# leggedrobotics/traversability_estimation

Measured on NVIDIA H100. Metric: Mcells/s full filter chain, synthetic elevation, higher is better.
Workload: dtype f32 (f64 certified slow path)

## Files before the change

### traversability_estimation_b200/csrc/te_capi.cu

```cuda
#include <cuda.h>
#include <cuda_runtime.h>

#include <cmath>
#include <cstdarg>
#include <cstdio>
#include <cstring>
#include <functional>
#include <map>
#include <mutex>
#include <string>
#include <vector>

#include "../../include/te_b200.h"
#include "te_kernels.h"
#include "te_fused.h"
#include "te_footprint.h"

namespace {

thread_local std::string g_last_error;

int fail(int code, const char* fmt, ...) {
  char buf[512];
  va_list ap;
// ... 207 lines not shown
  return TE_OK;
}

template <class F>
cudaError_t for_wrapped_pieces(int rows, int cols, int sr, int sc, int c0, int n, F&& copy) {
  for (int done = 0; done < n;) {
    const int c = c0 + done, js = (c + sc) % cols;
    const int m = std::min(n - done, cols - js);
    const size_t d = (size_t)c * rows, h = (size_t)js * rows;
    cudaError_t e = copy(d, h + sr, rows - sr, m);
    if (e == cudaSuccess && sr > 0) e = copy(d + (rows - sr), h, sr, m);
    if (e != cudaSuccess) return e;
    done += m;
  }
  return cudaSuccess;
}

cudaError_t upload_cols(float* dev, const float* host, int rows, int cols, int sr, int sc, int c0, int n, cudaStream_t s) {
  const size_t pitch = sizeof(float) * (size_t)rows;
  if (sr == 0 && sc == 0) return cudaMemcpyAsync(dev + (size_t)c0 * rows, host + (size_t)c0 * rows, pitch * n, cudaMemcpyHostToDevice, s);
  return for_wrapped_pieces(rows, cols, sr, sc, c0, n, [&](size_t d, size_t h, int r, int m) {
    return cudaMemcpy2DAsync(dev + d, pitch, host + h, pitch, sizeof(float) * r, m, cudaMemcpyHostToDevice, s);
  });
}

cudaError_t download_cols(float* host, const float* dev, int rows, int cols, int sr, int sc, int c0, int n, cudaStream_t s) {
  const size_t pitch = sizeof(float) * (size_t)rows;
  if (sr == 0 && sc == 0) return cudaMemcpyAsync(host + (size_t)c0 * rows, dev + (size_t)c0 * rows, pitch * n, cudaMemcpyDeviceToHost, s);
  return for_wrapped_pieces(rows, cols, sr, sc, c0, n, [&](size_t d, size_t h, int r, int m) {
    return cudaMemcpy2DAsync(host + h, pitch, dev + d, pitch, sizeof(float) * r, m, cudaMemcpyDeviceToHost, s);
  });
}

struct Staging {
  te_ctx* c;
  bool host;
  int rows, cols, sr, sc;
  int rc = TE_OK;
  int used = 0;
  struct Out { void* host; const void* dev; size_t bytes; int ncols; };
  Out outs[sizeof(te_ctx::stage) / sizeof(DevBuf)];
  int nout = 0;

  Staging(te_ctx* ctx, bool host_memory, const te_geometry* g)
      : c(ctx), host(host_memory), rows(g->rows), cols(g->cols), sr(g->start_row), sc(g->start_col) {}

  void check(cudaError_t e, const char* what) {
    if (rc == TE_OK && e != cudaSuccess) rc = fail(TE_ERR_CUDA, "%s failed: %s", what, cudaGetErrorString(e));
  }
  void* slot(size_t bytes) {
    if (rc != TE_OK) return nullptr;
    if (used == (int)(sizeof(outs) / sizeof(outs[0]))) {
      rc = fail(TE_ERR_CUDA, "out of staging buffers");
      return nullptr;
    }
    DevBuf& b = c->stage[used++];
    check(b.reserve(std::max<size_t>(bytes, 1)), "staging allocation");
    return rc == TE_OK ? b.p : nullptr;
  }
  size_t layer_bytes(int ncols) const { return sizeof(float) * (size_t)rows * ncols; }
  const float* in_layer(const float* h, int ncols) {
    if (!host || !h) return h;
    float* d = (float*)slot(layer_bytes(ncols));
    if (d) check(upload_cols(d, h, rows, cols, sr, sc, 0, ncols, c->stream), "layer upload");
    return d;
  }
  template <class T>
  const T* in(const T* h, size_t n) {
    if (!host || !h) return h;
    T* d = (T*)slot(sizeof(T) * n);
    if (d && n) check(cudaMemcpyAsync(d, h, sizeof(T) * n, cudaMemcpyHostToDevice, c->stream), "upload");
    return d;
  }
  float* out_layer(float* h, int ncols) { return (float*)record(h, layer_bytes(ncols), ncols); }
  template <class T>
  T* out(T* h, size_t n) { return (T*)record(h, sizeof(T) * n, 0); }
  void* record(void* h, size_t bytes, int ncols) {
    if (!host || !h) return h;
    void* d = slot(bytes);
    if (d) outs[nout++] = Out{h, d, bytes, ncols};
    return d;
  }
  int finish() {
    if (!host || rc != TE_OK) return rc;
    for (int k = 0; k < nout; ++k) {
      const Out& o = outs[k];
      check(o.ncols ? download_cols((float*)o.host, (const float*)o.dev, rows, cols, sr, sc, 0, o.ncols, c->stream)
                    : cudaMemcpyAsync(o.host, o.dev, o.bytes, cudaMemcpyDeviceToHost, c->stream),
            "download");
    }
    check(cudaStreamSynchronize(c->stream), "cudaStreamSynchronize");
    return rc;
  }
};

int next_timing_slot(te_ctx* c, te_ctx::Ev3** out) {
  if (c->events_used == c->events.size()) {
    te_ctx::Ev3 ev{};
    TE_CUDA(cudaEventCreate(&ev.a)); TE_CUDA(cudaEventCreate(&ev.b)); TE_CUDA(cudaEventCreate(&ev.c));
    c->events.push_back(ev);
  }
  *out = &c->events[c->events_used];
  return TE_OK;
}

int run_chain_device(te_ctx* c, const te_geometry* g, const te::SlabView& v, const te_chain_params* p, const float* elev,
                     const te::ChainOut& o, int nmaps) {
  const te::ChainDev d = make_chain_dev(g, p);
  bool use_fused = false;
  if (c->kernel_choice != TE_KERNEL_GENERIC) {
    use_fused = te::fused_eligible(c->fused, c->hX, c->hY, g, p, c->stream);
    if (!use_fused && c->kernel_choice == TE_KERNEL_FUSED)
      return fail(TE_ERR_UNSUPPORTED, "fused stencil has no instantiation for these window shapes: %s", c->fused.why.c_str());
    if (use_fused) {
      if (const char* why = te::fused_launch_obstacle(v, nmaps, elev, o)) {
        if (c->kernel_choice == TE_KERNEL_FUSED) return fail(TE_ERR_UNSUPPORTED, "fused stencil cannot run this launch: %s", why);
        use_fused = false;
      }
    }
  }
  const size_t in_stride = (size_t)g->rows * v.in_ncols, out_stride = (size_t)g->rows * v.out_ncols;
  if (use_fused) {
    const size_t cells = out_stride * (size_t)nmaps;
    const size_t cap = te::fused_list_capacity(cells, c->sms);
    if (cap >= ((size_t)1 << 32)) return fail(TE_ERR_UNSUPPORTED, "launch of %zu cells exceeds the work-list index range", cells);
    TE_CUDA(c->worklist.reserve(sizeof(unsigned) * cap));
    TE_CUDA(c->worklist3.reserve(sizeof(unsigned) * cells));
    {
      const void* before = c->counter.p;
      TE_CUDA(c->counter.reserve(sizeof(unsigned) * 256));
      if (c->counter.p != before) c->counter_clean = -1;
    }
    {
      const te::ChainOut& om = o;
      const int phase = c->counter_phase ^ 1;
      unsigned* const cnt = (unsigned*)c->counter.p + 128 * phase;
      unsigned* const cnt_next = (unsigned*)c->counter.p + 128 * (phase ^ 1);
      if (c->counter_stream != c->stream) c->counter_clean = -1;
      c->counter_stream = c->stream;
      if (c->counter_clean != phase) TE_CUDA(cudaMemsetAsync(cnt, 0, sizeof(unsigned) * 128, c->stream));
      c->counter_clean = -1;
      c->counter_phase = phase;
      te_ctx::Ev3* ev = nullptr;
      if (c->timing) {
        if (int rc = next_timing_slot(c, &ev)) return rc;
        TE_CUDA(cudaEventRecord(ev->a, c->stream));
      }
      int rc = te::launch_chain_fused(c->fused, v, d, nmaps, elev, om, (unsigned*)c->worklist.p, cnt, (unsigned)cap, c->sms, c->stream);
      if (rc != 0) return fail(TE_ERR_CUDA, "fused chain launch failed: %s", c->fused.why.c_str());
      if (int r2 = launch_check(c, "k_chain_fused")) return r2;
      if (c->timing) TE_CUDA(cudaEventRecord(ev->b, c->stream));
      te::FixupArgs fa;
      te::make_fixup_args(c->fused, v, d, &fa);
      te::launch_fixup_t2(fa, elev, om, (const unsigned*)c->worklist.p, cnt, (unsigned)cap, (unsigned*)c->worklist3.p, cnt + 4,
                          (unsigned)cells, c->sms, c->stream, !c->timing);
      if (int r2 = launch_check(c, "k_fixup_t2")) return r2;
      te::launch_fixup(v, d, elev, om, (const unsigned*)c->worklist3.p, cnt + 4, (unsigned)cells, cnt_next, c->sms, c->stream, true);
      if (int r2 = launch_check(c, "k_fixup_cells")) return r2;
      c->counter_clean = phase ^ 1;
      if (c->timing) {
        TE_CUDA(cudaEventRecord(ev->c, c->stream));
        ++c->events_used;
      }
    }
  } else {
    for (int m = 0; m < nmaps; ++m) {
      te::ChainOut om = o;
      om.slope += m * out_stride; om.step += m * out_stride; om.rough += m * out_stride; om.trav += m * out_stride;
      if (om.nx) om.nx += m * out_stride;
      if (om.ny) om.ny += m * out_stride;
      if (om.nz) om.nz += m * out_stride;
      te_ctx::Ev3* ev = nullptr;
      if (c->timing) {
        if (int rc = next_timing_slot(c, &ev)) return rc;
        TE_CUDA(cudaEventRecord(ev->a, c->stream));
      }
      te::launch_chain_generic(v, d, elev + m * in_stride, om, c->sms, c->stream);
      if (int r2 = launch_check(c, "k_chain_generic")) return r2;
      if (c->timing) {
        TE_CUDA(cudaEventRecord(ev->b, c->stream));
        TE_CUDA(cudaEventRecord(ev->c, c->stream));
        ++c->events_used;
      }
    }
  }
  return TE_OK;
}

}

extern "C" {

int te_abi_version(void) { return TE_B200_ABI_VERSION; }

const char* te_last_error(void) { return g_last_error.c_str(); }

int te_create(te_ctx** out, int device) {
  if (!out) return fail(TE_ERR_BAD_ARG, "out pointer is null");
  *out = nullptr;
  int n = 0;
  cudaError_t e = cudaGetDeviceCount(&n);
  if (e != cudaSuccess || n <= 0)
    return fail(TE_ERR_CUDA, "no CUDA device available (%s); libte_b200 has no CPU fallback", e == cudaSuccess ? "device count 0" : cudaGetErrorString(e));
  if (device < 0 || device >= n) return fail(TE_ERR_BAD_ARG, "device %d out of range [0,%d)", device, n);
  int prev = 0;
  cudaGetDevice(&prev);
  TE_CUDA(cudaSetDevice(device));
  te_ctx* c = new te_ctx();
  c->device = device;
  cudaDeviceProp prop;
  if (cudaGetDeviceProperties(&prop, device) == cudaSuccess) c->sms = prop.multiProcessorCount;
  e = cudaStreamCreateWithFlags(&c->own_stream, cudaStreamNonBlocking);
  if (e != cudaSuccess) {
    delete c;
    cudaSetDevice(prev);
    return fail(TE_ERR_CUDA, "cudaStreamCreate failed: %s", cudaGetErrorString(e));
  }
  c->stream = c->own_stream;
  cudaSetDevice(prev);
  *out = c;
  return TE_OK;
}

int te_destroy(te_ctx* c) {
  if (!c) return TE_OK;
  {
    Guard g(c);
    if (g.ok) {
      cudaStreamSynchronize(c->stream);
      c->dX.release();
      c->dY.release();
      for (auto& b : c->stage) b.release();
      c->worklist.release();
      c->worklist3.release();
      c->counter.release();
      c->fused.release();
      c->fp.release();
      for (auto& e : c->events) { cudaEventDestroy(e.a); cudaEventDestroy(e.b); cudaEventDestroy(e.c); }
      if (c->s_h2d) cudaStreamDestroy(c->s_h2d);
      if (c->s_d2h) cudaStreamDestroy(c->s_d2h);
      if (c->own_stream) cudaStreamDestroy(c->own_stream);
    }
  }
  delete c;
  return TE_OK;
}

int te_host_alloc(void** out, size_t bytes) {
  if (!out) return fail(TE_ERR_BAD_ARG, "out pointer is null");
  *out = nullptr;
  TE_CUDA(cudaHostAlloc(out, bytes ? bytes : 1, cudaHostAllocDefault));
  return TE_OK;
}

int te_host_free(void* p) {
  if (!p) return TE_OK;
  TE_CUDA(cudaFreeHost(p));
  return TE_OK;
}

int te_set_stream(te_ctx* c, void* s) {
  TE_ENTER(c);
  c->stream = s ? (cudaStream_t)s : c->own_stream;
  return TE_OK;
}

int te_synchronize(te_ctx* c) {
  TE_ENTER(c);
  TE_CUDA(cudaStreamSynchronize(c->stream));
  return TE_OK;
}

int te_set_kernel(te_ctx* c, int choice) {
  TE_ENTER(c);
  if (choice < TE_KERNEL_AUTO || choice > TE_KERNEL_FUSED) return fail(TE_ERR_BAD_ARG, "unknown kernel choice %d", choice);
  c->kernel_choice = choice;
  return TE_OK;
}

int te_get_stats(te_ctx* c, int64_t* launches, int64_t* slow) {
  TE_ENTER(c);
  if (launches) *launches = c->launches;
  if (slow) {
    unsigned last[4] = {0, 0, 0, 0};
    if (c->counter.p) {
      TE_CUDA(cudaStreamSynchronize(c->stream));
      TE_CUDA(cudaMemcpy(last, (unsigned*)c->counter.p + 128 * c->counter_phase, sizeof(last), cudaMemcpyDeviceToHost));
    }
    *slow = (int64_t)last[1];
  }
  return TE_OK;
}

int te_enable_timing(te_ctx* c, int on) {
  TE_ENTER(c);
  c->timing = on != 0;
  return TE_OK;
}

int te_get_timing(te_ctx* c, double* main_ms, double* fixup_ms, int64_t* samples) {
  TE_ENTER(c);
  TE_CUDA(cudaStreamSynchronize(c->stream));
  double m = 0.0, f = 0.0;
  for (size_t k = 0; k < c->events_used; ++k) {
    const auto& e = c->events[k];
    float t1 = 0.f, t2 = 0.f;
    TE_CUDA(cudaEventElapsedTime(&t1, e.a, e.b));
    TE_CUDA(cudaEventElapsedTime(&t2, e.b, e.c));
// ... 1054 lines not shown
```

### traversability_estimation_b200/csrc/te_fixup.cu

```cuda
#include <algorithm>

#include "te_fused.h"

namespace te {
namespace {

struct Elev {
  const float* __restrict__ e;
  int rows, col0, ncols, cols_total;
  __device__ __forceinline__ float operator()(int a, int b) const {
    if (a < 0 || a >= rows || b < 0 || b >= cols_total) return nanf_();
    const int lb = b - col0;
    if (lb < 0 || lb >= ncols) return nanf_();
    const float v = __ldg(e + (size_t)lb * rows + a);
    return finitef(v) ? v : nanf_();
  }
};

__device__ float step_height_t2(const FixupArgs& A, const Elev& E, int a, int b) {
  const float zc = E(a, b);
  if (!finitef(zc)) return nanf_();
  const unsigned rm = A.rowmask ? A.rowmask[a] : 0u, cm = A.colmask ? A.colmask[b] : 0u;
  float mn = zc, mx = zc;
#pragma unroll
  for (int l = -2; l <= 2; ++l) {
    const int w = A.w1[l < 0 ? -l : l];
    for (int k = -w; k <= w; ++k) {
      const float z = E(a + k, b + l);
      if (finitef(z)) { mn = fminf(mn, z); mx = fmaxf(mx, z); }
    }
  }
  if (A.tip1) {
    const float t0 = (rm & 1u) ? E(a - 2, b) : nanf_(), t1 = (rm & 2u) ? E(a + 2, b) : nanf_();
    const float t2 = (cm & 1u) ? E(a, b - 2) : nanf_(), t3 = (cm & 2u) ? E(a, b + 2) : nanf_();
    mn = fminf(fminf(mn, t0), fminf(t1, fminf(t2, t3)));
    mx = fmaxf(fmaxf(mx, t0), fmaxf(t1, fmaxf(t2, t3)));
  }
  return (float)((double)mx - (double)mn);
}

__device__ __noinline__ float step_t2(const FixupArgs A, const Elev E, int i, int j) {
  const unsigned rm = A.rowmask ? A.rowmask[i] : 0u, cm = A.colmask ? A.colmask[j] : 0u;
  double stepMax = 0.0;
  int n = 0;
  bool any = false;
  auto visit = [&](int a, int b) {
    const float sh = step_height_t2(A, E, a, b);
    if (!finitef(sh)) return;
    any = true;
    if ((double)sh > stepMax) stepMax = (double)sh;
    if ((double)sh > A.step_crit) ++n;
  };
  for (int l = -2; l <= 2; ++l) {
    const int w = A.w2[l < 0 ? -l : l];
    for (int k = -w; k <= w; ++k) visit(i + k, j + l);
  }
  if (A.tip2) {
    if (rm & 4u) visit(i - 2, j);
    if (rm & 8u) visit(i + 2, j);
    if (cm & 4u) visit(i, j - 2);
    if (cm & 8u) visit(i, j + 2);
  }
  if (!any) return nanf_();
  const double step = fmin(stepMax, (double)n / (double)A.ncrit * stepMax);
  return (float)(step < A.step_crit ? 1.0 - step / A.step_crit : 0.0);
}

__constant__ double c_rcp[26] = {0.0,      1.0 / 1,  1.0 / 2,  1.0 / 3,  1.0 / 4,  1.0 / 5,  1.0 / 6,  1.0 / 7,  1.0 / 8,
                                 1.0 / 9,  1.0 / 10, 1.0 / 11, 1.0 / 12, 1.0 / 13, 1.0 / 14, 1.0 / 15, 1.0 / 16, 1.0 / 17,
                                 1.0 / 18, 1.0 / 19, 1.0 / 20, 1.0 / 21, 1.0 / 22, 1.0 / 23, 1.0 / 24, 1.0 / 25};

__device__ __forceinline__ float acos_t2(float x) {
  const float u = 1.0f - x;
  float p = fmaf(x, -0.0011488182935863733f, 0.006254698149859905f);
  p = fmaf(p, x, -0.016484638676047325f);
  p = fmaf(p, x, 0.03044925443828106f);
  p = fmaf(p, x, -0.05000271648168564f);
  p = fmaf(p, x, 0.08894557505846024f);
  p = fmaf(p, x, -0.21459604799747467f);
  p = fmaf(p, x, 1.570796251296997f);
  return sqrtf(u) * p;
}

constexpr unsigned shape_mask(int w0, int w1, int w2) {
  auto col = [](int w) { return w >= 2 ? 0x1fu : w == 1 ? 0x0eu : w == 0 ? 0x04u : 0u; };
  return (col(w2)) | (col(w1) << 5) | (col(w0) << 10) | (col(w1) << 15) | (col(w2) << 20);
}
constexpr unsigned SHAPE_A = shape_mask(2, 2, 1), SHAPE_B = shape_mask(1, 1, -1);

template <unsigned SHAPE>
__device__ bool normals_t2(const FixupArgs& A, const Elev& E, int i, int j, float& fnx, float& fny, float& fnz, float& slope,
                           float& rough, unsigned& why) {
  const float zc = E(i, j);
  if (!finitef(zc)) {
    fnx = fny = fnz = slope = rough = nanf_();
    return true;
  }
  unsigned mask = 0;
  double sw = 0, suw = 0, svw = 0, sww = 0;
  {
    const int lb0 = j - A.in_col0;
    const double dzc = (double)zc;
    unsigned shape = SHAPE;
    if (SHAPE == 0u) {
#pragma unroll
      for (int l = -2; l <= 2; ++l) {
        const int w = A.wn[l < 0 ? -l : l];
        shape |= (w >= 2 ? 0x1fu : w == 1 ? 0x0eu : w == 0 ? 0x04u : 0u) << ((l + 2) * 5);
      }
    }
    float v[5][5];
    if (i >= 2 && i + 2 < A.rows && j >= 2 && j + 2 < A.cols_total && lb0 >= 2 && lb0 + 2 < A.in_ncols) {
      const float* base = E.e + (size_t)lb0 * A.rows + i;
#pragma unroll
      for (int l = -2; l <= 2; ++l)
#pragma unroll
        for (int k = -2; k <= 2; ++k)
          v[l + 2][k + 2] = (SHAPE == 0u || ((SHAPE >> ((l + 2) * 5 + (k + 2))) & 1u)) ? __ldg(base + (ptrdiff_t)l * A.rows + k) : 0.0f;
    } else {
#pragma unroll
      for (int l = -2; l <= 2; ++l) {
        const int b = j + l, lb = lb0 + l;
        const bool col_ok = b >= 0 && b < A.cols_total && lb >= 0 && lb < A.in_ncols;
        const float* col = E.e + (size_t)min(max(lb, 0), A.in_ncols - 1) * A.rows;
#pragma unroll
        for (int k = -2; k <= 2; ++k) {
          const int a = i + k;
          if (SHAPE != 0u && !((SHAPE >> ((l + 2) * 5 + (k + 2))) & 1u)) { v[l + 2][k + 2] = 0.0f; continue; }
          const float x = __ldg(col + min(max(a, 0), A.rows - 1));
          v[l + 2][k + 2] = (col_ok && a >= 0 && a < A.rows) ? x : nanf_();
        }
      }
    }
#pragma unroll
    for (int l = -2; l <= 2; ++l) {
      double cs = 0.0, ck = 0.0;
#pragma unroll
      for (int k = -2; k <= 2; ++k) {
        const unsigned bitm = 1u << ((l + 2) * 5 + (k + 2));
        if (SHAPE != 0u && !(SHAPE & bitm)) continue;
        const bool ok = finitef(v[l + 2][k + 2]) && (shape & bitm) != 0u;
        mask |= ok ? bitm : 0u;
        const double d = (double)(ok ? v[l + 2][k + 2] : zc) - dzc;
        cs += d;
        if (k != 0) ck = fma((double)k, d, ck);
        sww = fma(d, d, sww);
      }
      sw += cs;
      suw += ck;
      if (l != 0) svw = fma((double)l, cs, svw);
    }
    suw *= -A.res;
    svw *= -A.res;
  }
  constexpr unsigned KM = 0x108421u, LM = 0x1fu;
  const int k_m2 = __popc(mask & KM), k_m1 = __popc(mask & (KM << 1)), k_p1 = __popc(mask & (KM << 3)), k_p2 = __popc(mask & (KM << 4));
  const int l_m2 = __popc(mask & LM), l_m1 = __popc(mask & (LM << 5)), l_p1 = __popc(mask & (LM << 15)), l_p2 = __popc(mask & (LM << 20));
  auto bit = [](int k, int l) { return 1u << ((l + 2) * 5 + (k + 2)); };
  const unsigned kl_p1 = bit(1, 1) | bit(-1, -1), kl_m1 = bit(1, -1) | bit(-1, 1);
  const unsigned kl_p2 = bit(2, 1) | bit(1, 2) | bit(-2, -1) | bit(-1, -2), kl_m2 = bit(2, -1) | bit(-1, 2) | bit(-2, 1) | bit(1, -2);
  const unsigned kl_p4 = bit(2, 2) | bit(-2, -2), kl_m4 = bit(2, -2) | bit(-2, 2);
  const int ik = 2 * (k_p2 - k_m2) + (k_p1 - k_m1), il = 2 * (l_p2 - l_m2) + (l_p1 - l_m1);
  const int ikk = 4 * (k_p2 + k_m2) + (k_p1 + k_m1), ill = 4 * (l_p2 + l_m2) + (l_p1 + l_m1);
  const int ikl = (__popc(mask & kl_p1) - __popc(mask & kl_m1)) + 2 * (__popc(mask & kl_p2) - __popc(mask & kl_m2)) +
                  4 * (__popc(mask & kl_p4) - __popc(mask & kl_m4));
  const double res2 = A.res * A.res;
  const int cnt = __popc(mask);
  const double su = -A.res * (double)ik, sv = -A.res * (double)il;
  const double suu = res2 * (double)ikk, svv = res2 * (double)ill, suv = res2 * (double)ikl;
  double nx = 0.0, ny = 0.0, nz = 1.0;
  const double rn = c_rcp[cnt];
  const double mu = su * rn, mv = sv * rn, mw = sw * rn;
  const double xx = fma(-su, mu, suu), xy = fma(-su, mv, suv), xz = fma(-su, mw, suw);
  const double yy = fma(-sv, mv, svv), yz = fma(-sv, mw, svw), zz = fma(-sw, mw, sww);
  if (cnt >= 3 && zz > 0.0) {
    double bx, by, bz;
    if (cnt == A.n_full_i) {
      const double a = 0.5 * (xx + yy), g2 = fma(xz, xz, yz * yz);
      const double h = 0.5 * (a - zz), hh = fma(h, h, g2);
      const double D = sqrt(hh);
      const double dph = D + fabs(h);
      why = 1u | ((unsigned)cnt << 8);
      if (!(dph > 0.0)) return false;
      const double qq = g2 / dph;
      const double m = h >= 0.0 ? dph : qq;
      const double lam = (h >= 0.0 ? zz : a) - qq;
      const double big = fmax(a, zz);
      why = 2u | ((unsigned)cnt << 8);
      if (!(lam > 1e-9 * big)) return false;
      why = 3u | ((unsigned)cnt << 8);
      if (!(fmin(2.0 * D, m) > 1e-7 * big)) return false;
      bx = -xz; by = -yz; bz = m;
    } else {
      const double c2 = xx + yy + zz;
      const double c1 = xx * yy + xx * zz + yy * zz - xy * xy - xz * xz - yz * yz;
      const double c0 = xx * (yy * zz - yz * yz) - xy * (xy * zz - yz * xz) + xz * (xy * yz - yy * xz);
      double lam = 0.0, dp = -c1;
      bool conv = false;
#pragma unroll 1
      for (int it = 0; it < 40; ++it) {
        const double pv = fma(fma(c2 - lam, lam, -c1), lam, c0);
        dp = fma(fma(-3.0, lam, 2.0 * c2), lam, -c1);
        const double hpp = fma(-3.0, lam, c2);
        const double den = fma(dp, dp, -pv * hpp);
        if (!(den > 0.0)) break;
        const double step = pv * dp / den;
        lam -= step;
        if (fabs(step) <= 1e-15 * c2) { conv = true; break; }
      }
      dp = fma(fma(-3.0, lam, 2.0 * c2), lam, -c1);
      why = (!conv ? 4u : !(lam > 1e-9 * c2) ? 5u : 6u) | ((unsigned)cnt << 8);
      if (!conv || !(lam > 1e-9 * c2) || !(fabs(dp) > 1e-4 * c2 * c2)) return false;
      const double ax = xx - lam, ay = yy - lam, az = zz - lam;
      const double v0x = xy * yz - xz * ay, v0y = xz * xy - ax * yz, v0z = ax * ay - xy * xy;
      const double v1x = xy * az - xz * yz, v1y = xz * xz - ax * az, v1z = ax * yz - xy * xz;
      const double v2x = ay * az - yz * yz, v2y = yz * xz - xy * az, v2z = xy * yz - ay * xz;
      const double q0 = v0x * v0x + v0y * v0y + v0z * v0z, q1 = v1x * v1x + v1y * v1y + v1z * v1z, q2 = v2x * v2x + v2y * v2y + v2z * v2z;
      bx = v0x; by = v0y; bz = v0z;
      double bq = q0;
      if (q1 > bq) { bx = v1x; by = v1y; bz = v1z; bq = q1; }
      if (q2 > bq) { bx = v2x; by = v2y; bz = v2z; bq = q2; }
    }
    const double bq = fma(bx, bx, fma(by, by, bz * bz));
    why = 7u | ((unsigned)cnt << 8);
    if (!(bq > 0.0)) return false;
    const double inv = rsqrt(bq);
    nx = bx * inv; ny = by * inv; nz = bz * inv;
    if (nz < 0.0) { nx = -nx; ny = -ny; nz = -nz; }
    why = 8u | ((unsigned)cnt << 8);
    if (nz == 0.0) return false;
    if (nz > 0.9998) {
      const float f = (float)nz;
      const float up = __uint_as_float(__float_as_uint(f) + 1u), dn = __uint_as_float(__float_as_uint(f) - 1u);
      const double bu = 0.5 * ((double)f + (double)up), bd = 0.5 * ((double)f + (double)dn);
      const double guard = A.nz_guard * (bu - bd);
      why = 9u | ((unsigned)cnt << 8);
      if (fabs(nz - bu) < guard || fabs(nz - bd) < guard) return false;
    }
  }
  fnx = (float)nx; fny = (float)ny; fnz = (float)nz;
  const double th = (double)acos_t2(fminf(fnz, 1.0f));
  slope = (float)(th < A.slope_crit ? fma(-th, A.inv_slope_crit, 1.0) : 0.0);
  const double NX = fnx, NY = fny, NZ = fnz;
  const double sum = fmax(NX * (NX * xx + 2.0 * (NY * xy + NZ * xz)) + NY * (NY * yy + 2.0 * NZ * yz) + NZ * NZ * zz, 0.0);
  if (cnt >= 2) {
    const double r = sqrt(sum * c_rcp[cnt - 1]);
    rough = (float)(r < A.rough_crit ? fma(-r, A.inv_rough_crit, 1.0) : 0.0);
  } else {
    rough = 0.0f;
  }
  return true;
}

template <unsigned SHAPE>
__global__ void __launch_bounds__(128, 8) k_fixup_t2(FixupArgs A, const float* __restrict__ elev, ChainOut o,
                                                  const unsigned* __restrict__ list, const unsigned* __restrict__ count,
                                                  unsigned cap, unsigned* list3, unsigned* count3, unsigned cap3) {
  asm volatile("griddepcontrol.launch_dependents;");
  asm volatile("griddepcontrol.wait;" ::: "memory");
  unsigned n = *count;
  if (n > cap) n = cap;
  for (unsigned k = blockIdx.x * blockDim.x + threadIdx.x; k < n; k += gridDim.x * blockDim.x) {
    const unsigned w = list[k];
    if (w == LIST_INVALID) continue;
    const unsigned c = w & 0x3fffffffu;
    const unsigned mapi = c / A.map_cells, cl = c - mapi * A.map_cells;
    const int i = (int)(cl % (unsigned)A.rows);
    const int j = A.out_col0 + (int)(cl / (unsigned)A.rows);
    const Elev E{elev + (size_t)mapi * A.in_map_stride, A.rows, A.in_col0, A.in_ncols, A.cols_total};
    const bool do_n = (w >> 30) & 1u, do_s = (w >> 31) & 1u;
    float s, r, t;
    bool escalate = false;
    unsigned why = 0;
    if (do_n) {
      float fx, fy, fz;
      if (normals_t2<SHAPE>(A, E, i, j, fx, fy, fz, s, r, why)) {
        o.slope[c] = s;
        o.rough[c] = r;
        if (o.nx) { o.nx[c] = fx; o.ny[c] = fy; o.nz[c] = fz; }
      } else {
        escalate = true;
      }
    } else {
      s = o.slope[c];
      r = o.rough[c];
    }
    if (do_s) {
      t = step_t2(A, E, i, j);
      o.step[c] = t;
    } else {
      t = o.step[c];
    }
    if (escalate) {
      const unsigned idx = atomicAdd(count3, 1u);
      if (idx < cap3) list3[idx] = c | (1u << 30);
      else atomicExch(count3 + 1, 1u);
      atomicAdd(count3 + 4 + (why & 15u), 1u);
      atomicAdd(count3 + 20 + min((why >> 8) & 31u, 25u), 1u);
    } else {
      o.trav[c] = __fmul_rn(A.fuse_w, __fadd_rn(__fadd_rn(s, t), r));
    }
  }
}

}

void launch_fixup_t2(const FixupArgs& a, const float* elev, const ChainOut& o, const unsigned* list, const unsigned* count,
                     unsigned cap, unsigned* list3, unsigned* count3, unsigned cap3, int sms, cudaStream_t s, bool pdl) {
  cudaLaunchConfig_t cfg{};
  const unsigned long long want = ((unsigned long long)cap3 / 32ull + 127ull) / 128ull;
  cfg.gridDim = dim3((unsigned)std::min<unsigned long long>((unsigned long long)sms * 64ull, std::max<unsigned long long>(want, (unsigned long long)sms * 2ull)));
  cfg.blockDim = dim3(128);
  cfg.stream = s;
  cudaLaunchAttribute at{};
  at.id = cudaLaunchAttributeProgrammaticStreamSerialization;
  at.val.programmaticStreamSerializationAllowed = 1;
  cfg.attrs = &at;
  cfg.numAttrs = pdl ? 1 : 0;
  const bool is_a = a.wn[0] == 2 && a.wn[1] == 2 && a.wn[2] == 1, is_b = a.wn[0] == 1 && a.wn[1] == 1 && a.wn[2] == -1;
  if (is_a) cudaLaunchKernelEx(&cfg, k_fixup_t2<SHAPE_A>, a, elev, o, list, count, cap, list3, count3, cap3);
  else if (is_b) cudaLaunchKernelEx(&cfg, k_fixup_t2<SHAPE_B>, a, elev, o, list, count, cap, list3, count3, cap3);
  else cudaLaunchKernelEx(&cfg, k_fixup_t2<0u>, a, elev, o, list, count, cap, list3, count3, cap3);
}

}
```

### traversability_estimation_b200/csrc/te_fused.h

```cpp
#pragma once
#include <cuda_runtime.h>
#include <string>
#include <vector>
#include "../../include/te_b200.h"
#include "te_kernels.h"

namespace te {

struct FusedState {
  std::string why;
  bool valid = false;
  te_geometry key_geo{};
  te_chain_params key_par{};
  int shape_id = -1;
  std::vector<unsigned char> h_rowmask, h_colmask;
  DevBuf rowmask, colmask;
  bool smem_attr[4] = {false, false, false, false};
  void invalidate() { valid = false; }
  void release();
};

bool fused_eligible(FusedState& st, const std::vector<double>& X, const std::vector<double>& Y, const te_geometry* g,
                    const te_chain_params* p, cudaStream_t stream);
const char* fused_launch_obstacle(const SlabView& v, int nmaps, const float* elev, const ChainOut& o);

struct FixupArgs {
  int rows, cols_total, in_col0, in_ncols, out_col0;
  unsigned map_cells;
  size_t in_map_stride;
  int wn[3], w1[3], w2[3];
  int tip1, tip2;
  int ncrit;
  double n_full;
  int n_full_i;
  double res, slope_crit, step_crit, rough_crit;
  double inv_slope_crit, inv_rough_crit;
  double nz_guard;
  float fuse_w;
  const unsigned char* rowmask;
  const unsigned char* colmask;
};

void make_fixup_args(const FusedState& st, const SlabView& v, const ChainDev& p, FixupArgs* out);
void launch_fixup_t2(const FixupArgs& a, const float* elev, const ChainOut& o, const unsigned* list, const unsigned* count,
                     unsigned cap, unsigned* list3, unsigned* count3, unsigned cap3, int sms, cudaStream_t s, bool pdl);

constexpr unsigned LIST_INVALID = 0xffffffffu;
size_t fused_list_capacity(size_t cells, int sms);

void fused_plan(int rows, int out_ncols, int nmaps, int sms, int out[19]);

int launch_chain_fused(FusedState& st, const SlabView& v, const ChainDev& p, int nmaps, const float* elev, const ChainOut& o,
                       unsigned* list, unsigned* count, unsigned cap, int sms, cudaStream_t s);

}
```

Baseline: 70850.

## Compact fixup worklist per warp and vectorise stencil loads in tier-2 fixup

Reworks the tier-2 fixup kernel so each warp collects valid worklist entries into a shared-memory queue via ballot before processing, which cuts divergence from invalid slots. The 5x5 normal window is now read as aligned float4 pairs, and the runtime-shape template variant is removed. The grid is sized from an occupancy query, launch bounds are relaxed, and the eigen/normal arithmetic is rewritten with explicit FMAs. Any other window shape, or a row count not divisible by 4, now returns an error instead of running. The FMA rewrites can change rounding relative to the certified reference path.

Result: no change. 71530, median of 6 (+1.0%).

```diff
diff --git a/traversability_estimation_b200/csrc/te_capi.cu b/traversability_estimation_b200/csrc/te_capi.cu
--- a/traversability_estimation_b200/csrc/te_capi.cu
+++ b/traversability_estimation_b200/csrc/te_capi.cu
@@ -383,8 +383,12 @@
       if (c->timing) TE_CUDA(cudaEventRecord(ev->b, c->stream));
       te::FixupArgs fa;
       te::make_fixup_args(c->fused, v, d, &fa);
-      te::launch_fixup_t2(fa, elev, om, (const unsigned*)c->worklist.p, cnt, (unsigned)cap, (unsigned*)c->worklist3.p, cnt + 4,
-                          (unsigned)cells, c->sms, c->stream, !c->timing);
+      const cudaError_t e2 = te::launch_fixup_t2(fa, elev, om, (const unsigned*)c->worklist.p, cnt, (unsigned)cap,
+                                                 (unsigned*)c->worklist3.p, cnt + 4, (unsigned)cells, c->sms, c->stream, !c->timing);
+      if (e2 != cudaSuccess) {
+        cudaGetLastError();
+        return fail(TE_ERR_CUDA, "k_fixup_t2 launch failed: %s", cudaGetErrorString(e2));
+      }
       if (int r2 = launch_check(c, "k_fixup_t2")) return r2;
       te::launch_fixup(v, d, elev, om, (const unsigned*)c->worklist3.p, cnt + 4, (unsigned)cells, cnt_next, c->sms, c->stream, true);
       if (int r2 = launch_check(c, "k_fixup_cells")) return r2;
diff --git a/traversability_estimation_b200/csrc/te_fixup.cu b/traversability_estimation_b200/csrc/te_fixup.cu
--- a/traversability_estimation_b200/csrc/te_fixup.cu
+++ b/traversability_estimation_b200/csrc/te_fixup.cu
@@ -1,5 +1,3 @@
-#include <algorithm>
-
 #include "te_fused.h"
 
 namespace te {
@@ -39,7 +37,8 @@
   return (float)((double)mx - (double)mn);
 }
 
-__device__ __noinline__ float step_t2(const FixupArgs A, const Elev E, int i, int j) {
+__device__ __noinline__ float step_t2(const FixupArgs& A, const float* e, int i, int j) {
+  const Elev E{e, A.rows, A.in_col0, A.in_ncols, A.cols_total};
   const unsigned rm = A.rowmask ? A.rowmask[i] : 0u, cm = A.colmask ? A.colmask[j] : 0u;
   double stepMax = 0.0;
   int n = 0;
@@ -89,34 +88,29 @@
 constexpr unsigned SHAPE_A = shape_mask(2, 2, 1), SHAPE_B = shape_mask(1, 1, -1);
 
 template <unsigned SHAPE>
-__device__ bool normals_t2(const FixupArgs& A, const Elev& E, int i, int j, float& fnx, float& fny, float& fnz, float& slope,
-                           float& rough, unsigned& why) {
-  const float zc = E(i, j);
-  if (!finitef(zc)) {
-    fnx = fny = fnz = slope = rough = nanf_();
-    return true;
-  }
+__device__ __forceinline__ bool normals_t2(const FixupArgs& A, const Elev& E, int i, int j, float& fnx, float& fny, float& fnz,
+                                           float& slope, float& rough, unsigned& why) {
+  static_assert(SHAPE != 0u && ((SHAPE >> 12) & 1u), "the window shape is a compile-time constant and holds its centre");
   unsigned mask = 0;
   double sw = 0, suw = 0, svw = 0, sww = 0;
   {
     const int lb0 = j - A.in_col0;
-    const double dzc = (double)zc;
-    unsigned shape = SHAPE;
-    if (SHAPE == 0u) {
-#pragma unroll
-      for (int l = -2; l <= 2; ++l) {
-        const int w = A.wn[l < 0 ? -l : l];
-        shape |= (w >= 2 ? 0x1fu : w == 1 ? 0x0eu : w == 0 ? 0x04u : 0u) << ((l + 2) * 5);
-      }
-    }
     float v[5][5];
     if (i >= 2 && i + 2 < A.rows && j >= 2 && j + 2 < A.cols_total && lb0 >= 2 && lb0 + 2 < A.in_ncols) {
-      const float* base = E.e + (size_t)lb0 * A.rows + i;
-#pragma unroll
-      for (int l = -2; l <= 2; ++l)
+      const int a0 = (i - 2) & ~3, r = (i - 2) - a0;
+      const float* base = E.e + (size_t)lb0 * A.rows + a0;
+#pragma unroll
+      for (int l = -2; l <= 2; ++l) {
+        if (!((SHAPE >> ((l + 2) * 5)) & 0x1fu)) continue;
+        const float4* col = reinterpret_cast<const float4*>(base + (ptrdiff_t)l * A.rows);
+        const float4 p = __ldg(col), q = __ldg(col + 1);
+        const float x[8] = {p.x, p.y, p.z, p.w, q.x, q.y, q.z, q.w};
 #pragma unroll
         for (int k = -2; k <= 2; ++k)
-          v[l + 2][k + 2] = (SHAPE == 0u || ((SHAPE >> ((l + 2) * 5 + (k + 2))) & 1u)) ? __ldg(base + (ptrdiff_t)l * A.rows + k) : 0.0f;
+          v[l + 2][k + 2] = ((SHAPE >> ((l + 2) * 5 + (k + 2))) & 1u)
+                                ? (r == 0 ? x[k + 2] : r == 1 ? x[k + 3] : r == 2 ? x[k + 4] : x[k + 5])
+                                : 0.0f;
+      }
     } else {
 #pragma unroll
       for (int l = -2; l <= 2; ++l) {
@@ -126,20 +120,26 @@
 #pragma unroll
         for (int k = -2; k <= 2; ++k) {
           const int a = i + k;
-          if (SHAPE != 0u && !((SHAPE >> ((l + 2) * 5 + (k + 2))) & 1u)) { v[l + 2][k + 2] = 0.0f; continue; }
+          if (!((SHAPE >> ((l + 2) * 5 + (k + 2))) & 1u)) { v[l + 2][k + 2] = 0.0f; continue; }
           const float x = __ldg(col + min(max(a, 0), A.rows - 1));
           v[l + 2][k + 2] = (col_ok && a >= 0 && a < A.rows) ? x : nanf_();
         }
       }
     }
+    const float zc = v[2][2];
+    if (!finitef(zc)) {
+      fnx = fny = fnz = slope = rough = nanf_();
+      return true;
+    }
+    const double dzc = (double)zc;
 #pragma unroll
     for (int l = -2; l <= 2; ++l) {
       double cs = 0.0, ck = 0.0;
 #pragma unroll
       for (int k = -2; k <= 2; ++k) {
         const unsigned bitm = 1u << ((l + 2) * 5 + (k + 2));
-        if (SHAPE != 0u && !(SHAPE & bitm)) continue;
-        const bool ok = finitef(v[l + 2][k + 2]) && (shape & bitm) != 0u;
+        if (!(SHAPE & bitm)) continue;
+        const bool ok = finitef(v[l + 2][k + 2]);
         mask |= ok ? bitm : 0u;
         const double d = (double)(ok ? v[l + 2][k + 2] : zc) - dzc;
         cs += d;
@@ -193,8 +193,8 @@
       bx = -xz; by = -yz; bz = m;
     } else {
       const double c2 = xx + yy + zz;
-      const double c1 = xx * yy + xx * zz + yy * zz - xy * xy - xz * xz - yz * yz;
-      const double c0 = xx * (yy * zz - yz * yz) - xy * (xy * zz - yz * xz) + xz * (xy * yz - yy * xz);
+      const double c1 = fma(-yz, yz, fma(-xz, xz, fma(-xy, xy, fma(yy, zz, fma(xx, yy, xx * zz)))));
+      const double c0 = fma(xz, fma(xy, yz, -(yy * xz)), fma(xx, fma(yy, zz, -(yz * yz)), -(xy * fma(xy, zz, -(yz * xz)))));
       double lam = 0.0, dp = -c1;
       bool conv = false;
 #pragma unroll 1
@@ -212,10 +212,11 @@
       why = (!conv ? 4u : !(lam > 1e-9 * c2) ? 5u : 6u) | ((unsigned)cnt << 8);
       if (!conv || !(lam > 1e-9 * c2) || !(fabs(dp) > 1e-4 * c2 * c2)) return false;
       const double ax = xx - lam, ay = yy - lam, az = zz - lam;
-      const double v0x = xy * yz - xz * ay, v0y = xz * xy - ax * yz, v0z = ax * ay - xy * xy;
-      const double v1x = xy * az - xz * yz, v1y = xz * xz - ax * az, v1z = ax * yz - xy * xz;
-      const double v2x = ay * az - yz * yz, v2y = yz * xz - xy * az, v2z = xy * yz - ay * xz;
-      const double q0 = v0x * v0x + v0y * v0y + v0z * v0z, q1 = v1x * v1x + v1y * v1y + v1z * v1z, q2 = v2x * v2x + v2y * v2y + v2z * v2z;
+      const double v0x = fma(xy, yz, -(xz * ay)), v0y = fma(xz, xy, -(ax * yz)), v0z = fma(ax, ay, -(xy * xy));
+      const double v1x = fma(xy, az, -(xz * yz)), v1y = fma(xz, xz, -(ax * az)), v1z = fma(-xy, xz, ax * yz);
+      const double v2x = fma(ay, az, -(yz * yz)), v2y = fma(-xy, az, yz * xz), v2z = fma(xy, yz, -(ay * xz));
+      const double q0 = fma(v0z, v0z, fma(v0x, v0x, v0y * v0y)), q1 = fma(v1z, v1z, fma(v1x, v1x, v1y * v1y));
+      const double q2 = fma(v2z, v2z, fma(v2x, v2x, v2y * v2y));
       bx = v0x; by = v0y; bz = v0z;
       double bq = q0;
       if (q1 > bq) { bx = v1x; by = v1y; bz = v1z; bq = q1; }
@@ -232,17 +233,17 @@
     if (nz > 0.9998) {
       const float f = (float)nz;
       const float up = __uint_as_float(__float_as_uint(f) + 1u), dn = __uint_as_float(__float_as_uint(f) - 1u);
-      const double bu = 0.5 * ((double)f + (double)up), bd = 0.5 * ((double)f + (double)dn);
-      const double guard = A.nz_guard * (bu - bd);
+      const double fu = (double)f + (double)up, bd = 0.5 * ((double)f + (double)dn);
+      const double guard = A.nz_guard * -fma(fu, -0.5, bd);
       why = 9u | ((unsigned)cnt << 8);
-      if (fabs(nz - bu) < guard || fabs(nz - bd) < guard) return false;
+      if (fabs(fma(fu, -0.5, nz)) < guard || fabs(nz - bd) < guard) return false;
     }
   }
   fnx = (float)nx; fny = (float)ny; fnz = (float)nz;
   const double th = (double)acos_t2(fminf(fnz, 1.0f));
   slope = (float)(th < A.slope_crit ? fma(-th, A.inv_slope_crit, 1.0) : 0.0);
   const double NX = fnx, NY = fny, NZ = fnz;
-  const double sum = fmax(NX * (NX * xx + 2.0 * (NY * xy + NZ * xz)) + NY * (NY * yy + 2.0 * NZ * yz) + NZ * NZ * zz, 0.0);
+  const double sum = fmax(fma(NZ * NZ, zz, fma(NY, fma(NY, yy, (2.0 * NZ) * yz), NX * fma(NX, xx, 2.0 * fma(NY, xy, NZ * xz)))), 0.0);
   if (cnt >= 2) {
     const double r = sqrt(sum * c_rcp[cnt - 1]);
     rough = (float)(r < A.rough_crit ? fma(-r, A.inv_rough_crit, 1.0) : 0.0);
@@ -252,75 +253,120 @@
   return true;
 }
 
+constexpr int T2_THREADS = 128;
+#ifndef TE_T2_MIN_BLOCKS
+#define TE_T2_MIN_BLOCKS 5
+#endif
+constexpr int T2_MIN_BLOCKS = TE_T2_MIN_BLOCKS;
+
 template <unsigned SHAPE>
-__global__ void __launch_bounds__(128, 8) k_fixup_t2(FixupArgs A, const float* __restrict__ elev, ChainOut o,
-                                                  const unsigned* __restrict__ list, const unsigned* __restrict__ count,
-                                                  unsigned cap, unsigned* list3, unsigned* count3, unsigned cap3) {
+__device__ __forceinline__ void fixup_cell(const FixupArgs& A, const float* __restrict__ elev, const ChainOut& o, unsigned w,
+                                           unsigned* list3, unsigned* count3, unsigned cap3) {
+  const unsigned c = w & 0x3fffffffu;
+  const unsigned mapi = c / A.map_cells, cl = c - mapi * A.map_cells;
+  const int i = (int)(cl % (unsigned)A.rows);
+  const int j = A.out_col0 + (int)(cl / (unsigned)A.rows);
+  const float* e = elev + (size_t)mapi * A.in_map_stride;
+  const bool do_n = (w >> 30) & 1u, do_s = (w >> 31) & 1u;
+  float s = 0.0f, r = 0.0f, t = 0.0f;
+  if (!do_n) { s = o.slope[c]; r = o.rough[c]; }
+  if (!do_s) t = o.step[c];
+  bool escalate = false;
+  unsigned why = 0;
+  if (do_n) {
+    float fx, fy, fz;
+    const Elev E{e, A.rows, A.in_col0, A.in_ncols, A.cols_total};
+    if (normals_t2<SHAPE>(A, E, i, j, fx, fy, fz, s, r, why)) {
+      o.slope[c] = s;
+      o.rough[c] = r;
+      if (o.nx) { o.nx[c] = fx; o.ny[c] = fy; o.nz[c] = fz; }
+    } else {
+      escalate = true;
+    }
+  }
+  if (do_s) {
+    t = step_t2(A, e, i, j);
+    o.step[c] = t;
+  }
+  if (escalate) {
+    const unsigned idx = atomicAdd(count3, 1u);
+    if (idx < cap3) list3[idx] = c | (1u << 30);
+    else atomicExch(count3 + 1, 1u);
+    atomicAdd(count3 + 4 + (why & 15u), 1u);
+    atomicAdd(count3 + 20 + min((why >> 8) & 31u, 25u), 1u);
+  } else {
+    o.trav[c] = __fmul_rn(A.fuse_w, __fadd_rn(__fadd_rn(s, t), r));
+  }
+}
+
+template <unsigned SHAPE>
+__global__ void __launch_bounds__(T2_THREADS, T2_MIN_BLOCKS)
+    k_fixup_t2(const __grid_constant__ FixupArgs A, const float* __restrict__ elev, const ChainOut o,
+               const unsigned* __restrict__ list, const unsigned* __restrict__ count, unsigned cap, unsigned* list3,
+               unsigned* count3, unsigned cap3) {
+  __shared__ unsigned queue[T2_THREADS / 32][64];
   asm volatile("griddepcontrol.launch_dependents;");
   asm volatile("griddepcontrol.wait;" ::: "memory");
   unsigned n = *count;
   if (n > cap) n = cap;
-  for (unsigned k = blockIdx.x * blockDim.x + threadIdx.x; k < n; k += gridDim.x * blockDim.x) {
-    const unsigned w = list[k];
-    if (w == LIST_INVALID) continue;
-    const unsigned c = w & 0x3fffffffu;
-    const unsigned mapi = c / A.map_cells, cl = c - mapi * A.map_cells;
-    const int i = (int)(cl % (unsigned)A.rows);
-    const int j = A.out_col0 + (int)(cl / (unsigned)A.rows);
-    const Elev E{elev + (size_t)mapi * A.in_map_stride, A.rows, A.in_col0, A.in_ncols, A.cols_total};
-    const bool do_n = (w >> 30) & 1u, do_s = (w >> 31) & 1u;
-    float s, r, t;
-    bool escalate = false;
-    unsigned why = 0;
-    if (do_n) {
-      float fx, fy, fz;
-      if (normals_t2<SHAPE>(A, E, i, j, fx, fy, fz, s, r, why)) {
-        o.slope[c] = s;
-        o.rough[c] = r;
-        if (o.nx) { o.nx[c] = fx; o.ny[c] = fy; o.nz[c] = fz; }
-      } else {
-        escalate = true;
-      }
-    } else {
-      s = o.slope[c];
-      r = o.rough[c];
-    }
-    if (do_s) {
-      t = step_t2(A, E, i, j);
-      o.step[c] = t;
-    } else {
-      t = o.step[c];
-    }
-    if (escalate) {
-      const unsigned idx = atomicAdd(count3, 1u);
-      if (idx < cap3) list3[idx] = c | (1u << 30);
-      else atomicExch(count3 + 1, 1u);
-      atomicAdd(count3 + 4 + (why & 15u), 1u);
-      atomicAdd(count3 + 20 + min((why >> 8) & 31u, 25u), 1u);
-    } else {
-      o.trav[c] = __fmul_rn(A.fuse_w, __fadd_rn(__fadd_rn(s, t), r));
-    }
-  }
-}
-
-}
-
-void launch_fixup_t2(const FixupArgs& a, const float* elev, const ChainOut& o, const unsigned* list, const unsigned* count,
-                     unsigned cap, unsigned* list3, unsigned* count3, unsigned cap3, int sms, cudaStream_t s, bool pdl) {
+  const unsigned lane = threadIdx.x & 31u;
+  unsigned* const q = queue[threadIdx.x >> 5];
+  const unsigned long long stride = (unsigned long long)gridDim.x * T2_THREADS;
+  unsigned long long base = (unsigned long long)blockIdx.x * T2_THREADS + (threadIdx.x & ~31u);
+  unsigned have = 0;
+  unsigned next = base + lane < n ? list[base + lane] : LIST_INVALID;
+  for (;;) {
+    while (have < 32u && base < n) {
+      const unsigned w = next;
+      base += stride;
+      next = base + lane < n ? list[base + lane] : LIST_INVALID;
+      const unsigned m = __ballot_sync(0xffffffffu, w != LIST_INVALID);
+      if (w != LIST_INVALID) q[have + __popc(m & ((1u << lane) - 1u))] = w;
+      have += __popc(m);
+    }
+    if (have == 0u) break;
+    __syncwarp();
+    const unsigned w = lane < have ? q[lane] : LIST_INVALID;
+    const unsigned rest = have > 32u ? have - 32u : 0u;
+    const unsigned keep = lane < rest ? q[32 + lane] : 0u;
+    __syncwarp();
+    if (lane < rest) q[lane] = keep;
+    have = rest;
+    if (w != LIST_INVALID) fixup_cell<SHAPE>(A, elev, o, w, list3, count3, cap3);
+  }
+}
+
+template <unsigned SHAPE>
+cudaError_t launch_t2(cudaLaunchConfig_t cfg, int sms, const FixupArgs& a, const float* elev, const ChainOut& o,
+                      const unsigned* list, const unsigned* count, unsigned cap, unsigned* list3, unsigned* count3, unsigned cap3) {
+  static const int per_sm = [] {
+    int nb = 0;
+    if (cudaOccupancyMaxActiveBlocksPerMultiprocessor(&nb, k_fixup_t2<SHAPE>, T2_THREADS, 0) != cudaSuccess) nb = 0;
+    return nb;
+  }();
+  if (per_sm <= 0) return cudaErrorInvalidConfiguration;
+  cfg.gridDim = dim3((unsigned)(per_sm * sms));
+  return cudaLaunchKernelEx(&cfg, k_fixup_t2<SHAPE>, a, elev, o, list, count, cap, list3, count3, cap3);
+}
+
+}
+
+cudaError_t launch_fixup_t2(const FixupArgs& a, const float* elev, const ChainOut& o, const unsigned* list, const unsigned* count,
+                            unsigned cap, unsigned* list3, unsigned* count3, unsigned cap3, int sms, cudaStream_t s, bool pdl) {
   cudaLaunchConfig_t cfg{};
-  const unsigned long long want = ((unsigned long long)cap3 / 32ull + 127ull) / 128ull;
-  cfg.gridDim = dim3((unsigned)std::min<unsigned long long>((unsigned long long)sms * 64ull, std::max<unsigned long long>(want, (unsigned long long)sms * 2ull)));
-  cfg.blockDim = dim3(128);
+  cfg.blockDim = dim3(T2_THREADS);
   cfg.stream = s;
   cudaLaunchAttribute at{};
   at.id = cudaLaunchAttributeProgrammaticStreamSerialization;
   at.val.programmaticStreamSerializationAllowed = 1;
   cfg.attrs = &at;
   cfg.numAttrs = pdl ? 1 : 0;
-  const bool is_a = a.wn[0] == 2 && a.wn[1] == 2 && a.wn[2] == 1, is_b = a.wn[0] == 1 && a.wn[1] == 1 && a.wn[2] == -1;
-  if (is_a) cudaLaunchKernelEx(&cfg, k_fixup_t2<SHAPE_A>, a, elev, o, list, count, cap, list3, count3, cap3);
-  else if (is_b) cudaLaunchKernelEx(&cfg, k_fixup_t2<SHAPE_B>, a, elev, o, list, count, cap, list3, count3, cap3);
-  else cudaLaunchKernelEx(&cfg, k_fixup_t2<0u>, a, elev, o, list, count, cap, list3, count3, cap3);
-}
-
-}
+  if ((a.rows & 3) != 0) return cudaErrorInvalidValue;
+  if (a.wn[0] == 2 && a.wn[1] == 2 && a.wn[2] == 1)
+    return launch_t2<SHAPE_A>(cfg, sms, a, elev, o, list, count, cap, list3, count3, cap3);
+  if (a.wn[0] == 1 && a.wn[1] == 1 && a.wn[2] == -1)
+    return launch_t2<SHAPE_B>(cfg, sms, a, elev, o, list, count, cap, list3, count3, cap3);
+  return cudaErrorInvalidValue;
+}
+
+}
diff --git a/traversability_estimation_b200/csrc/te_fused.h b/traversability_estimation_b200/csrc/te_fused.h
--- a/traversability_estimation_b200/csrc/te_fused.h
+++ b/traversability_estimation_b200/csrc/te_fused.h
@@ -42,8 +42,8 @@
 };
 
 void make_fixup_args(const FusedState& st, const SlabView& v, const ChainDev& p, FixupArgs* out);
-void launch_fixup_t2(const FixupArgs& a, const float* elev, const ChainOut& o, const unsigned* list, const unsigned* count,
-                     unsigned cap, unsigned* list3, unsigned* count3, unsigned cap3, int sms, cudaStream_t s, bool pdl);
+cudaError_t launch_fixup_t2(const FixupArgs& a, const float* elev, const ChainOut& o, const unsigned* list, const unsigned* count,
+                            unsigned cap, unsigned* list3, unsigned* count3, unsigned cap3, int sms, cudaStream_t s, bool pdl);
 
 constexpr unsigned LIST_INVALID = 0xffffffffu;
 size_t fused_list_capacity(size_t cells, int sms);
```
